# nv-tlabs/LION

Hardware: NVIDIA H100
Metric: shapes/sec (1000-step DDPM, 2048 latent pts, B=32) (higher is better)
Workload: dtype tf32 (fp32 storage/accumulate)

## Files before the change

include/lion_b200.h:

```cpp
#ifndef LION_B200_H
#define LION_B200_H
#include <stddef.h>
#ifdef __cplusplus
extern "C" {
#endif

typedef struct LionCtx LionCtx;
typedef struct LionModel LionModel;

int lion_version(void);
const char* lion_last_error(void);
int lion_ctx_create(int device, LionCtx** out);
int lion_ctx_destroy(LionCtx* ctx);
int lion_ctx_last_launches(LionCtx* ctx);
int lion_ctx_last_conv_group(LionCtx* ctx);
int lion_ctx_last_conv_stage_taps(LionCtx* ctx);
int lion_ctx_set_conv_whole_slabs(LionCtx* ctx, int on);
unsigned lion_ctx_generation(LionCtx* ctx);
int lion_ctx_timeline(LionCtx* ctx, unsigned long long* t_ns, char* names, int max_entries);
size_t lion_ctx_arena_bytes(LionCtx* ctx);
size_t lion_workspace_bytes(LionCtx* ctx);

int lion_avg_voxelize(const float* features, const int* coords, float* out, int* ind, int* cnt,
                      int B, int C, int N, int r, void* stream);
int lion_trilinear_devoxelize(const float* grid, const float* coords, float* out, int* inds, float* wgts,
                              int B, int C, int N, int r, int is_training, void* stream);
int lion_furthest_point_sampling(const float* coords, int* idx, int B, int N, int M, void* stream);
int lion_gather(const float* features, const int* idx, float* out, int B, int C, int N, int M, void* stream);
int lion_ball_query(const float* centers, const float* points, int* out, int B, int N, int M, float radius, int K,
                    void* stream);
int lion_grouping(const float* features, const int* idx, float* out, int B, int C, int N, int M, int U, void* stream);
int lion_three_nn_interpolate(const float* points, const float* centers, const float* centers_features, float* out,
                              int* idx, float* wgt, int B, int C, int N, int M, void* stream);
int lion_voxel_coords(const float* coords, float* norm_coords, int* vox, int B, int N, int r, int normalize, float eps,
                      void* stream);

int lion_avg_voxelize_backward(const float* grad_y , const int* ind , const int* cnt ,
                               float* grad_x , int B, int C, int N, int r, void* stream);
int lion_trilinear_devoxelize_backward(const float* grad_y , const int* inds , const float* wgts ,
                                       float* grad_x , int B, int C, int N, int r, void* stream);
int lion_grouping_backward(const float* grad_y , const int* idx , float* grad_x , int B, int C,
                           int N, int M, int U, void* stream);
int lion_three_nn_interpolate_backward(const float* grad_y , const int* idx , const float* wgt ,
                                       float* grad_x , int B, int C, int N, int M, void* stream);
int lion_gather_backward(const float* grad_y , const int* idx , float* grad_x , int B, int C, int N,
                         int M, void* stream);

enum { LION_KIND_UNET = 1, LION_KIND_PVCONV = 2, LION_KIND_SA = 3, LION_KIND_FP = 4, LION_KIND_ATTN = 5,
       LION_KIND_SHARED_MLP = 6, LION_KIND_GLOBAL_PRIOR = 7, LION_KIND_ADAGN = 8, LION_KIND_CONV3D = 9,
       LION_KIND_STYLE_ENC = 10 };
int lion_model_create(LionCtx* ctx, int kind, const int* desc, int ndesc, const float* const* params, int nparams,
                      LionModel** out);
int lion_model_destroy(LionModel* m);
int lion_model_refresh(LionModel* m);

int lion_unet_forward(LionModel* m, const float* x, const float* t, const float* style, const float* clip, float* out,
                      int B, int N, void* stream);
#define LION_FWD_CONV_FP16 1
int lion_unet_forward_flags(LionModel* m, const float* x, const float* t, const float* style, const float* clip, float* out,
                            int B, int N, int flags, void* stream);
int lion_unet_cache_style(LionModel* m, const float* style, const float* clip, int B, void* stream);
int lion_style_encoder_forward(LionModel* m, const float* x, float* out, int B, int N, void* stream);
int lion_pvconv_fwd(LionModel* m, const float* features, const float* coords, const float* style, float* out,
                    int B, int N, void* stream);
int lion_sa_module_fwd(LionModel* m, const float* features, const float* coords, const float* style,
                       float* out_features, float* out_coords, int B, int N, void* stream);
int lion_fp_module_fwd(LionModel* m, const float* points_coords, const float* centers_coords,
                       const float* centers_features, const float* points_features, const float* style, float* out,
                       int B, int N, int M, void* stream);
int lion_linear_attention_fwd(LionModel* m, const float* x, float* out, int B, int N, void* stream);
// ... 67 lines not shown
```

lion_b200/_lib.py:

```python
import ctypes as C
import os
import threading

import torch

_HERE = os.path.dirname(os.path.abspath(__file__))
LIB_PATH = os.path.join(_HERE, "csrc", "liblion_b200.so")


class LionError(RuntimeError):
    pass


_lib = None
_lock = threading.Lock()
c_f = C.c_void_p


def _proto(lib):
    i, f, sz, vp = C.c_int, C.c_float, C.c_size_t, C.c_void_p
    P = lambda *a: list(a)
    sig = {
        "lion_version": ([], i),
        "lion_last_error": ([], C.c_char_p),
        "lion_ctx_create": (P(i, C.POINTER(vp)), i),
        "lion_ctx_destroy": (P(vp), i),
        "lion_ctx_last_launches": (P(vp), i),
        "lion_ctx_last_conv_group": (P(vp), i),
        "lion_ctx_last_conv_stage_taps": (P(vp), i),
        "lion_ctx_set_conv_whole_slabs": (P(vp, i), i),
        "lion_ctx_arena_bytes": (P(vp), sz),
        "lion_ctx_generation": (P(vp), C.c_uint),
        "lion_ctx_timeline": (P(vp, vp, vp, i), i),
        "lion_avg_voxelize": (P(vp, vp, vp, vp, vp, i, i, i, i, vp), i),
        "lion_trilinear_devoxelize": (P(vp, vp, vp, vp, vp, i, i, i, i, i, vp), i),
        "lion_furthest_point_sampling": (P(vp, vp, i, i, i, vp), i),
        "lion_gather": (P(vp, vp, vp, i, i, i, i, vp), i),
        "lion_ball_query": (P(vp, vp, vp, i, i, i, f, i, vp), i),
        "lion_grouping": (P(vp, vp, vp, i, i, i, i, i, vp), i),
        "lion_three_nn_interpolate": (P(vp, vp, vp, vp, vp, vp, i, i, i, i, vp), i),
        "lion_voxel_coords": (P(vp, vp, vp, i, i, i, i, f, vp), i),
        "lion_avg_voxelize_backward": (P(vp, vp, vp, vp, i, i, i, i, vp), i),
        "lion_trilinear_devoxelize_backward": (P(vp, vp, vp, vp, i, i, i, i, vp), i),
        "lion_grouping_backward": (P(vp, vp, vp, i, i, i, i, i, vp), i),
        "lion_three_nn_interpolate_backward": (P(vp, vp, vp, vp, i, i, i, i, vp), i),
        "lion_gather_backward": (P(vp, vp, vp, i, i, i, i, vp), i),
        "lion_model_create": (P(vp, i, C.POINTER(i), i, C.POINTER(vp), i, C.POINTER(vp)), i),
        "lion_model_destroy": (P(vp), i),
        "lion_model_refresh": (P(vp), i),
        "lion_unet_forward": (P(vp, vp, vp, vp, vp, vp, i, i, vp), i),
        "lion_unet_forward_flags": (P(vp, vp, vp, vp, vp, vp, i, i, i, vp), i),
        "lion_unet_cache_style": (P(vp, vp, vp, i, vp), i),
        "lion_style_encoder_forward": (P(vp, vp, vp, i, i, vp), i),
        "lion_pvconv_fwd": (P(vp, vp, vp, vp, vp, i, i, vp), i),
        "lion_sa_module_fwd": (P(vp, vp, vp, vp, vp, vp, i, i, vp), i),
        "lion_fp_module_fwd": (P(vp, vp, vp, vp, vp, vp, vp, i, i, i, vp), i),
        "lion_linear_attention_fwd": (P(vp, vp, vp, i, i, vp), i),
        "lion_shared_mlp_fwd": (P(vp, vp, vp, vp, i, i, vp), i),
        "lion_global_prior_forward": (P(vp, vp, vp, vp, vp, i, vp), i),
        "lion_adagn_fwd": (P(vp, vp, vp, vp, i, i, vp), i),
        "lion_se3d_fwd": (P(vp, vp, vp, vp, vp, i, i, i, vp), i),
        "lion_swish_fwd": (P(vp, vp, sz, vp), i),
        "lion_ddpm_update": (P(vp, vp, vp, vp, vp, vp, f, sz, vp, i, vp), i),
        "lion_ddpm_set_step": (P(vp, vp, i, i, vp), i),
        "lion_ddpm_next_step": (P(vp, vp, i, vp), i),
        "lion_ddpm_fetch_noise": (P(vp, vp, vp, sz, vp), i),
        "lion_conv3d_gn_fwd": (P(vp, vp, vp, vp, vp, i, vp), i),
        "lion_conv3d_gn_fwd_flags": (P(vp, vp, vp, vp, vp, i, i, vp), i),
        "lion_pvconv_conv1_probe": (P(vp, vp, vp, i, vp, vp, vp, C.POINTER(i), i, i, vp), i),
        "lion_sa_mlp_probe": (P(vp, vp, vp, vp, i, vp, vp, vp, vp, vp, vp, C.POINTER(i), i, i, vp), i),
        "lion_pvconv_probe": (P(vp, vp, vp, vp, vp, vp, vp, vp, vp, vp, vp, vp, C.POINTER(i), i, i, vp), i),
        "lion_pvconv_probe_flags": (P(vp, vp, vp, vp, vp, vp, vp, vp, vp, vp, vp, vp, C.POINTER(i), i, i, i, vp), i),
        "lion_attention_probe": (P(vp, vp, vp, vp, vp, i, i, vp), i),
        "lion_global_prior_step": (P(vp, vp, vp, vp, vp, i, vp), i),
        "lion_workspace_bytes": (P(vp), sz),
        "lion_ddim_update": (P(vp, vp, vp, vp, vp, vp, sz, vp, vp), i),
        "lion_ddim_set_step": (P(vp, vp, vp, i, i, i, vp), i),
        "lion_ddim_next_step": (P(vp, vp, vp, i, i, vp), i),
        "lion_scheduler_step": (P(vp, vp, vp, vp, vp, vp, sz, vp), i),
        "lion_chamfer_forward": (P(vp, vp, vp, vp, vp, vp, i, i, i, vp), i),
        "lion_chamfer_pairwise": (P(vp, vp, vp, i, i, i, i, vp), i),
        "lion_chamfer_backward": (P(vp, vp, vp, vp, vp, vp, vp, vp, i, i, i, vp), i),
        "lion_emd_approx": (P(vp, vp, vp, i, i, i, vp), i),
# ... 174 lines not shown
```

lion_b200/csrc/common.cuh:

```cuda
#pragma once
#include <cuda_runtime.h>
#include <cstdint>
#include <cstdio>
#include <cstdarg>
#include <cstring>
#include <string>
#include <vector>
#include <mutex>

namespace lion {

enum : int { LION_OK = 0, LION_ERR_CUDA = -1, LION_ERR_ARG = -2, LION_ERR_OOM = -3, LION_ERR_STATE = -4 };

void set_error(const char* fmt, ...);
const char* get_error();

#define LION_CHECK_CUDA(expr)                                                          \
  do {                                                                                 \
    cudaError_t _e = (expr);                                                           \
    if (_e != cudaSuccess) {                                                           \
      lion::set_error("%s:%d: %s -> %s", __FILE__, __LINE__, #expr, cudaGetErrorString(_e)); \
      return lion::LION_ERR_CUDA;                                                      \
    }                                                                                  \
  } while (0)

#define LION_REQUIRE(cond, ...)                                                        \
  do {                                                                                 \
    if (!(cond)) {                                                                     \
      lion::set_error(__VA_ARGS__);                                                    \
      return lion::LION_ERR_ARG;                                                       \
    }                                                                                  \
  } while (0)

#define LION_TRY(expr)                                                                 \
  do {                                                                                 \
    int _r = (expr);                                                                   \
    if (_r != 0) return _r;                                                            \
  } while (0)

constexpr int LION_MAX_STAMPS = 256;
struct Ctx {
  int device = 0;
  int num_sms = 132;
  int l2_bytes = 50 << 20;
  cudaStream_t stream = nullptr;
  cudaStream_t aux = nullptr;
  char* base = nullptr;
  char* zgrid = nullptr;
  size_t zgrid_cap = 0, zgrid_need = 0;
  size_t cap = 0;
  size_t off = 0;
  size_t peak = 0;
  unsigned generation = 0;
  std::mutex* mu = nullptr;
  bool dry = false;
  int launches = 0;
  int conv_smem_cap = 0;
  int conv_group_blocks = 0;
  int conv_stage_taps = 0;
  bool conv_whole_slabs = false;
  unsigned long long* d_stamps = nullptr;
  int n_stamps = 0;
  char stamp_names[LION_MAX_STAMPS][24];

  void reset() { off = 0; peak = 0; launches = 0; zgrid_need = 0; n_stamps = 0; }
  void* alloc(size_t bytes) {
    size_t a = (off + 255) & ~size_t(255);
    off = a + bytes;
    if (off > peak) peak = off;
    if (dry) return (void*)(uintptr_t)(0x1000 + a);
    return base + a;
  }
  template <typename T> T* alloc_n(size_t n) { return (T*)alloc(n * sizeof(T)); }
  size_t mark() const { return off; }
  void release(size_t m) { off = m; }
};

int ctx_reserve(Ctx* c, size_t bytes);

#define LION_LAUNCH_ON(ctx, stream, kernel, grid, block, smem, ...)                    \
  do {                                                                                 \
    if (!(ctx)->dry) {                                                                 \
      kernel<<<(grid), (block), (smem), (stream)>>>(__VA_ARGS__);                      \
      (ctx)->launches++;                                                               \
    }                                                                                  \
  } while (0)
#define LION_LAUNCH(ctx, kernel, grid, block, smem, ...) LION_LAUNCH_ON(ctx, (ctx)->stream, kernel, grid, block, smem, __VA_ARGS__)

static __global__ void k_stamp(unsigned long long* p) {
  unsigned long long t;
  asm volatile("mov.u64 %0, %%globaltimer;" : "=l"(t));
  *p = t;
}
inline void stamp(Ctx* c, cudaStream_t s, const char* name, int idx = -1) {
  if (!c->d_stamps || c->dry || c->n_stamps >= LION_MAX_STAMPS) return;
  const char* pre = s == c->aux ? "aux:" : "";
  if (idx >= 0) snprintf(c->stamp_names[c->n_stamps], 24, "%s%s%d", pre, name, idx);
  else snprintf(c->stamp_names[c->n_stamps], 24, "%s%s", pre, name);
  k_stamp<<<1, 1, 0, s>>>(c->d_stamps + c->n_stamps);
  c->n_stamps++;
}

inline int memset_async(Ctx* c, void* p, int v, size_t bytes, cudaStream_t s) {
  if (c->dry || bytes == 0) return 0;
  LION_CHECK_CUDA(cudaMemsetAsync(p, v, bytes, s));
  return 0;
}
inline int memset_async(Ctx* c, void* p, int v, size_t bytes) { return memset_async(c, p, v, bytes, c->stream); }
inline int memcpy_d2d(Ctx* c, void* d, const void* s, size_t bytes) {
  if (c->dry || bytes == 0) return 0;
  LION_CHECK_CUDA(cudaMemcpyAsync(d, s, bytes, cudaMemcpyDeviceToDevice, c->stream));
  return 0;
}
// ... 62 lines not shown
```

lion_b200/csrc/conv_tc.cu:

```cuda
#include <algorithm>
#include <type_traits>
#include <cuda_fp16.h>

#include "common.cuh"
#include "model.cuh"
#include "wgmma.cuh"

namespace lion {
namespace tc {

using namespace sm90;

constexpr int CONSUMER_WARPS = 8;
constexpr int THREADS = 32 * CONSUMER_WARPS + 32;
__host__ __device__ constexpr int conv_threads(int BPW) { return BPW == 2 ? 32 * CONSUMER_WARPS + 128 : THREADS; }
constexpr int PRODUCER_REGS = 96, CONSUMER_REGS = 200;
constexpr int MAX_A_STAGES = 16;
constexpr int MAX_B_STAGES = 4;
constexpr int OCC_SMEM = 1024;
__host__ __device__ constexpr int tiles_per_item(int NT) { return NT <= 32 ? 4 : (NT <= 64 ? 2 : 1); }
constexpr int SMEM_BIAS = 128 * 4, SMEM_BARS = 64 * 8 + 128;
__host__ __device__ constexpr int smem_stat(int NT) { return CONSUMER_WARPS * 2 * NT * 4; }
__host__ __device__ constexpr int smem_pool(int NT, int TPG) { return TPG == 1 ? CONSUMER_WARPS * 2 * NT * 4 : 0; }
__host__ __device__ constexpr int smem_fixed(int NT, int TPG) {
  return SMEM_BIAS + smem_stat(NT) + smem_pool(NT, TPG) + SMEM_BARS + OCC_SMEM;
}

struct Params {
  const float4* in; const float* w; const float* bias; float4* out; double* ssum; double* ssq;
  int Gin, Gout_store, cout_pad;
  int rows;
  int p_begin, p_end;
  int ntile;
  int ntg, tpg;
  int tg_off[3];
  int tap_off[9];
  int r, rp, nzb, npl, nblk, ib;
  int halo;
  int KG, nchunk;
  int NT;
  int G;
  int B;
  int a_stage_bytes, b_stage_bytes, stage_rows;
  int a_stages;
  int b_stages;
  int tps;
  const unsigned char* occ;
  int occ_stride;
  float* pool_mm;
  int sched;
};

__host__ __device__ __forceinline__ int block_row(int k, int rp, int nzb, int npl) {
  const int x = k / npl, rem = k - x * npl, yb = rem / nzb, zb = rem - yb * nzb;
  return ((x + 1) * rp + 1 + 8 * yb) * rp + 1 + 8 * zb;
}

template <int KG, int TPG, int NT, int NB = 1, typename OP = float>
__device__ __forceinline__ void issue_stage(float (*d)[NT / 2], const uint32_t* a_addr, uint32_t b_addr, uint32_t a_pitch,
                                            uint32_t a_sbo, const int* tap_off) {
  const uint64_t b0 = make_desc(b_addr, NT * 16, 128);
  uint64_t a0[NB];
#pragma unroll
  for (int k = 0; k < NB; ++k) a0[k] = make_desc(a_addr[k], a_pitch, a_sbo);
#pragma unroll
  for (int t = 0; t < TPG; ++t) {
    const uint64_t toff = (uint64_t)(int64_t)(TPG == 1 ? 0 : tap_off[t]);
#pragma unroll
    for (int ks = 0; ks < KG / 2; ++ks)
#pragma unroll
      for (int k = 0; k < NB; ++k) {
        const uint64_t a = a0[k] + toff + (uint64_t)((ks * 2 * a_pitch) >> 4), b = b0 + (uint64_t)(((t * KG + ks * 2) * NT * 16) >> 4);
        if constexpr (std::is_same<OP, __half>::value) wgmma_f16<NT>(d[k], a, b, 1);
        else wgmma_tf32<NT>(d[k], a, b, 1);
      }
  }
}


struct Items {
  long long u, u_end; int ntile_total, B, G;
  int mode, m, q, n_p, n_q, c_i, i, big, k;
  __device__ __forceinline__ bool next(int& nt, long long& v0, int& ntile) {
    const long long per_nt = (long long)B * ntile_total;
    if (mode) {
      while (u >= u_end) {
        if (k >= m) return false;
        const int a0 = q * k / m, a1 = q * (k + 1) / m, b0 = (q + 1) * k / m, b1 = (q + 1) * (k + 1) / m;
        u = (long long)n_q * a0 + (long long)n_p * b0 + (long long)(i - c_i) * (a1 - a0) + (long long)c_i * (b1 - b0);
        u_end = u + (big ? b1 - b0 : a1 - a0);
        ++k;
      }
      nt = (int)(u / per_nt);
      v0 = u - (long long)nt * per_nt;
      const long long lim = (long long)(nt + 1) * per_nt;
      const long long e = u_end < lim ? u_end : lim;
      ntile = (int)(e - u);
      u = e;
      return true;
    }
    if (u >= u_end) return false;
    nt = (int)(u / per_nt);
    v0 = u - (long long)nt * per_nt;
    long long run = per_nt - v0;
    if (u_end - u < run) run = u_end - u;
    const long long k2 = (run + G - 1) / G;
    ntile = (int)((run + k2 - 1) / k2);
    u += ntile;
    return true;
  }
};
__device__ __forceinline__ Items make_items(long long U, int ntile_total, int B, int G, int sched) {
  const long long u_begin = U * blockIdx.x / gridDim.x, u_end = U * (blockIdx.x + 1) / gridDim.x;
  Items it{u_begin, u_end, ntile_total, B, G, 0, 0, 0, 0, 0, 0, 0, 0, 0};
  if (sched) {
    const int grid = (int)gridDim.x, q = (int)(U / grid), n_p = (int)(U - (long long)q * grid);
    const int tmax = q + (n_p ? 1 : 0);
    it.mode = 1; it.u = 0; it.u_end = 0;
    it.m = (tmax + G - 1) / G; it.q = q; it.n_p = n_p; it.n_q = grid - n_p;
    it.i = (int)blockIdx.x; it.c_i = (int)(u_begin - (long long)q * blockIdx.x);
    it.big = (int)(u_end - u_begin) > q; it.k = 0;
  }
  return it;
}

__device__ __forceinline__ void halo_mask(int p_lo, int rp, bool& ok_lo, bool& ok_hi) {
  const int p_hi = p_lo + 8;
  const int z0 = p_lo % rp, y0 = (p_lo / rp) % rp, z1 = p_hi % rp, y1 = (p_hi / rp) % rp;
  ok_lo = ok_lo && z0 >= 1 && z0 <= rp - 2 && y0 >= 1 && y0 <= rp - 2;
  ok_hi = ok_hi && z1 >= 1 && z1 <= rp - 2 && y1 >= 1 && y1 <= rp - 2;
}
template <int NT>
__device__ __forceinline__ void stat_add(float* s_stat, int cw, int lane, int col, float x0, float x1, float x2, float x3) {
  const float s0 = red8<0>(x0 + x2), s1 = red8<0>(x1 + x3);
  const float q0 = red8<0>(fmaf(x0, x0, x2 * x2)), q1 = red8<0>(fmaf(x1, x1, x3 * x3));
  if (lane < 4) {
    float* st = s_stat + (cw * 2) * NT + col;
    st[0] += s0; st[1] += s1; st[NT] += q0; st[NT + 1] += q1;
  }
}
template <int NT>
__device__ __forceinline__ void stat_flush(const Params& P, float* s_stat, int et, int b, int n0) {
  asm volatile("bar.sync 1, 256;" ::: "memory");
  if (et < NT) {
    float s = 0.f, qq = 0.f;
#pragma unroll
    for (int w = 0; w < CONSUMER_WARPS; ++w) {
      s += s_stat[(w * 2 + 0) * NT + et]; qq += s_stat[(w * 2 + 1) * NT + et];
      s_stat[(w * 2 + 0) * NT + et] = 0.0f; s_stat[(w * 2 + 1) * NT + et] = 0.0f;
    }
    atomicAdd(P.ssum + (size_t)b * P.cout_pad + n0 + et, (double)s);
    atomicAdd(P.ssq + (size_t)b * P.cout_pad + n0 + et, (double)qq);
  }
  asm volatile("bar.sync 1, 256;" ::: "memory");
}

template <int KG, int TPG, int NT, bool BLK, int BPW = 1, int TPS = TPG, typename OP = float>
__global__ void __launch_bounds__(conv_threads(BPW), 1) k_conv_tc(Params P) {
  constexpr int GT = BLK ? BPW : tiles_per_item(NT);
  constexpr int NTHR = conv_threads(BPW);
  constexpr bool SETREG = NTHR > THREADS;
  constexpr int NACC = NT / 2;
  constexpr int NPARTS = TPG / TPS;
  extern __shared__ __align__(128) uint8_t smem[];
  uint8_t* sA = smem;
  const int A_STAGES = P.a_stages;
  uint8_t* sB = sA + (size_t)A_STAGES * P.a_stage_bytes;
  const int B_STAGES = P.b_stages;
  float* s_bias = (float*)(sB + (size_t)B_STAGES * P.b_stage_bytes);
  float* s_stat = s_bias + 128;
  float* s_pool = s_stat + CONSUMER_WARPS * 2 * NT;
  uint64_t* bars = (uint64_t*)((uint8_t*)s_stat + smem_stat(NT) + smem_pool(NT, TPG));
  volatile uint32_t* s_skip = (volatile uint32_t*)(bars + 64);
  uint8_t* s_occ = (uint8_t*)(bars + 64) + 128;
  const int tid = threadIdx.x, warp = tid >> 5, lane = tid & 31;

  const uint32_t bar_full_a = smem_u32(bars), bar_empty_a = smem_u32(bars + MAX_A_STAGES);
  const uint32_t bar_full_b = smem_u32(bars + 2 * MAX_A_STAGES), bar_empty_b = smem_u32(bars + 2 * MAX_A_STAGES + MAX_B_STAGES);

  if (P.Gin % KG != 0)
    for (int i = tid; i < A_STAGES * P.a_stage_bytes / 16; i += NTHR) ((float4*)sA)[i] = make_float4(0.f, 0.f, 0.f, 0.f);
  for (int i = tid; i < CONSUMER_WARPS * 2 * NT; i += NTHR) s_stat[i] = 0.0f;
  if (tid == 0) {
    for (int i = 0; i < A_STAGES; ++i) { mbar_init(bar_full_a + 8 * i, 1); mbar_init(bar_empty_a + 8 * i, CONSUMER_WARPS); }
    for (int i = 0; i < B_STAGES; ++i) { mbar_init(bar_full_b + 8 * i, 1); mbar_init(bar_empty_b + 8 * i, CONSUMER_WARPS); }
    asm volatile("fence.mbarrier_init.release.cluster;" ::: "memory");
  }
  asm volatile("fence.proxy.async.shared::cta;" ::: "memory");
  __syncthreads();

  const int ntile_total = P.ntile;
  const int n_nt = P.cout_pad / P.NT;
  const long long U = (long long)n_nt * P.B * ntile_total;
  const Items items0 = make_items(U, ntile_total, P.B, P.G, P.sched);

  if (warp >= CONSUMER_WARPS) {
    if constexpr (SETREG) {
      regs_dec<PRODUCER_REGS>();
      if (warp > CONSUMER_WARPS) return;
    }
    uint32_t sa = 0, pa = 0, sb = 0, pb = 0;
    const uint32_t bytes = (uint32_t)P.stage_rows * 16u;
    const uint32_t sA_addr = smem_u32(sA), sB_addr = smem_u32(sB);
    Items items = items0;
    int nt, ntile;
    long long v0;
    int occ_shape = -1;
    const int slab_floats = P.tpg * KG * NT * 4;
    auto copy_weights = [&](const float* src) {
      mbar_wait<SETREG>(bar_empty_b + 8 * sb, pb ^ 1);
      if (lane == 0) {
        mbar_expect_tx(bar_full_b + 8 * sb, P.b_stage_bytes);
        bulk_g2s(sB_addr + sb * (uint32_t)P.b_stage_bytes, src, P.b_stage_bytes, bar_full_b + 8 * sb);
      }
      if (++sb == B_STAGES) { sb = 0; pb ^= 1; }
// ... 10 lines not shown
          const float* slab = wsrc + (size_t)(cc * P.ntg + tg) * slab_floats;
          copy_weights(slab);
          for (int j = 0; j < ntile; ++j) {
            const int bj = __shfl_sync(0xffffffffu, my_b, j), tj = __shfl_sync(0xffffffffu, my_t, j);
            long long row0;
            uint32_t cnt = (uint32_t)P.stage_rows;
            if (!BLK) {
              row0 = (long long)P.p_begin + (long long)tj * 128 - P.halo + P.tg_off[tg];
            } else {
              row0 = (long long)block_row(tj * P.ib, P.rp, P.nzb, P.npl) - P.rp - 1 + P.tg_off[tg];
              if (row0 + cnt > (long long)P.rows) cnt = (uint32_t)(P.rows - row0);
            }
            const float4* in_lane = P.in + ((size_t)bj * P.Gin + grp_lane) * P.rows;
            mbar_wait<SETREG>(bar_empty_a + 8 * sa, pa ^ 1);
            bool empty = false;
            if (may_skip) {
              const unsigned char* occ_b = P.occ + (size_t)bj * P.occ_stride;
              if (P.occ_stride <= OCC_SMEM) {
                if (occ_shape != bj) {
                  __syncwarp();
                  for (int k = lane; k < P.occ_stride; k += 32) s_occ[k] = __ldg(occ_b + k);
                  __syncwarp();
                  occ_shape = bj;
                }
                occ_b = s_occ;
              }
              long long lo = row0 < 0 ? 0 : row0, hi = row0 + cnt - 1;
              if (hi > P.rows - 1) hi = P.rows - 1;
              unsigned any = 0;
              for (int k = (int)(lo >> 6); k <= (int)(hi >> 6); ++k) any |= occ_b[k];
              empty = (any == 0);
            }
            const uint32_t full = bar_full_a + 8 * sa;
            if (lane == 0) {
              s_skip[sa] = empty ? 1u : 0u;
              if (empty) asm volatile("mbarrier.arrive.release.cta.shared::cta.b64 _, [%0];" ::"r"(full) : "memory");
              else mbar_expect_tx(full, cnt * 16u * kg_real);
            }
            __syncwarp();
            if (!empty && lane < kg_real)
              bulk_g2s(sA_addr + sa * (uint32_t)P.a_stage_bytes + lane * bytes, in_lane + row0, cnt * 16u, full);
            if (++sa == (uint32_t)A_STAGES) { sa = 0; pa ^= 1; }
          }
          for (int s = 1; s < NPARTS; ++s) copy_weights(slab + (size_t)s * (P.b_stage_bytes / 4));
        }
      }
    }
  } else {
    if constexpr (SETREG) regs_inc<CONSUMER_REGS>();
    const int cw = warp, wg = cw >> 2, wq = cw & 3;
    const int et = tid;
    const uint32_t a_pitch = (uint32_t)P.stage_rows * 16u;
    const uint32_t a_sbo = BLK ? (uint32_t)P.rp * 16u : 128u;
    const uint32_t a_ring = smem_u32(sA) + (BLK ? 0u : (uint32_t)(P.halo + 64 * wg) * 16u);
    const uint32_t b_ring = smem_u32(sB);
    const int r_lo = 64 * wg + 16 * wq + (lane >> 2);
    const int c_lo = 2 * (lane & 3);
    const bool odd = (lane & 1) != 0;
    float acc[GT][NACC];
    uint32_t sa = 0, pa = 0, sb = 0, pb = 0;
    Items items = items0;
    int nt, ntile;
    long long v0;
    auto release = [&](int& s, uint32_t bar0) {
      if (s >= 0) { if (lane == 0) mbar_arrive(bar0 + 8 * s); s = -1; }
    };
    while (items.next(nt, v0, ntile)) {
#pragma unroll
      for (int j = 0; j < GT; ++j)
#pragma unroll
        for (int i = 0; i < NACC; ++i) acc[j][i] = 0.0f;
      int g_f = 0, nbw = 0;
      uint32_t boff[GT];
      if (BLK) {
        const int g_b = (int)(v0 / ntile_total);
        g_f = (int)(v0 - (long long)g_b * ntile_total) * P.ib;
        const int nb = min(P.ib, P.nblk - g_f);
        nbw = (nb - wg + 1) / 2;
        const int s_f = block_row(g_f, P.rp, P.nzb, P.npl);
#pragma unroll
        for (int j = 0; j < GT; ++j) {
          const int k = 2 * j + wg < nb ? g_f + 2 * j + wg : g_f;
          boff[j] = (uint32_t)(block_row(k, P.rp, P.nzb, P.npl) - s_f + P.rp + 1) * 16u;
        }
      }
      int pend_a = -1, pend_b = -1;
      bool skip[BLK ? 1 : GT];
      for (int cc = 0; cc < P.nchunk; ++cc) {
        for (int tg = 0; tg < P.ntg; ++tg) {
          const uint32_t sa0 = sa, pa0 = pa;
#pragma unroll
          for (int s = 0; s < NPARTS; ++s) {
            mbar_wait<SETREG>(bar_full_b + 8 * sb, pb);
            const uint32_t b_addr = b_ring + sb * (uint32_t)P.b_stage_bytes;
            const int* toff = P.tap_off + s * TPS;
            bool issued = false;
            sa = sa0; pa = pa0;
#pragma unroll
            for (int j = 0; j < (BLK ? 1 : GT); ++j) {
              if (j < ntile) {
                if (s == 0) {
                  mbar_wait<SETREG>(bar_full_a + 8 * sa, pa);
                  skip[j] = s_skip[sa] != 0;
                  if (skip[j]) { int st = (int)sa; release(st, bar_empty_a); }
                }
                if (!skip[j]) {
                  const uint32_t a_addr = a_ring + sa * (uint32_t)P.a_stage_bytes;
                  wg_fence();
                  if (!BLK) {
                    issue_stage<KG, TPS, NT, 1, OP>(&acc[j], &a_addr, b_addr, a_pitch, a_sbo, toff);
                  } else {
                    uint32_t a_blk[GT];
#pragma unroll
                    for (int k = 0; k < GT; ++k) a_blk[k] = a_addr + boff[k];
                    issue_stage<KG, TPS, NT, GT, OP>(acc, a_blk, b_addr, a_pitch, a_sbo, toff);
                  }
                  wg_commit();
                  wg_wait<1>();
                  release(pend_a, bar_empty_a);
                  release(pend_b, bar_empty_b);
                  if (s == NPARTS - 1) pend_a = (int)sa;
                  issued = true;
                }
                if (++sa == (uint32_t)A_STAGES) { sa = 0; pa ^= 1; }
              }
            }
            if (pend_b >= 0) {
              wg_wait<0>();
              release(pend_a, bar_empty_a);
              release(pend_b, bar_empty_b);
            }
            if (issued) pend_b = (int)sb;
            else { int st = (int)sb; release(st, bar_empty_b); }
            if (++sb == B_STAGES) { sb = 0; pb ^= 1; }
          }
        }
      }
      wg_wait<0>();
      release(pend_a, bar_empty_a);
      release(pend_b, bar_empty_b);
#pragma unroll
      for (int j = 0; j < GT; ++j) fence_regs<NACC>(acc[j]);

      const int n0 = nt * NT;
      asm volatile("bar.sync 1, 256;" ::: "memory");
      if (et < NT) s_bias[et] = P.bias ? P.bias[n0 + et] : 0.0f;
      asm volatile("bar.sync 1, 256;" ::: "memory");
      int b = (int)(v0 / ntile_total);
#pragma unroll
      for (int j = 0; j < GT; ++j) {
        if (j < (BLK ? nbw : ntile)) {
          int tj = 0, p_lo, p_hi;
          bool ok_lo, ok_hi;
          bool in_lo, in_hi;
          if (!BLK) {
            const long long vj = v0 + j;
            const int bj = (int)(vj / ntile_total);
            tj = (int)(vj - (long long)bj * ntile_total);
            if (bj != b) { if (P.ssum) stat_flush<NT>(P, s_stat, et, b, n0); b = bj; }
            p_lo = P.p_begin + tj * 128 + r_lo; p_hi = p_lo + 8;
            in_lo = p_lo < P.p_end; in_hi = p_hi < P.p_end;
            ok_lo = in_lo; ok_hi = in_hi;
            if (TPG != 1) halo_mask(p_lo, P.rp, ok_lo, ok_hi);
          } else {
            const int k = g_f + 2 * j + wg, x = k / P.npl, rem = k - x * P.npl, yb = rem / P.nzb, zb = rem - yb * P.nzb;
            const int y = 1 + 8 * yb + 2 * wq, z = 1 + 8 * zb + (lane >> 2);
            p_lo = ((x + 1) * P.rp + y) * P.rp + z; p_hi = p_lo + P.rp;
            ok_lo = y <= P.r && z <= P.r; ok_hi = y + 1 <= P.r && z <= P.r;
            in_lo = ok_lo; in_hi = ok_hi;
          }
#pragma unroll
          for (int i = 0; i < NT / 8; ++i) {
            const int col = 8 * i + c_lo;
            const float x0 = ok_lo ? acc[j][4 * i + 0] + s_bias[col] : 0.0f, x1 = ok_lo ? acc[j][4 * i + 1] + s_bias[col + 1] : 0.0f;
            const float x2 = ok_hi ? acc[j][4 * i + 2] + s_bias[col] : 0.0f, x3 = ok_hi ? acc[j][4 * i + 3] + s_bias[col + 1] : 0.0f;
            if (P.ssum) stat_add<NT>(s_stat, cw, lane, col, x0, x1, x2, x3);
            if (TPG == 1 && P.pool_mm) {
              const float mn0 = red8<1>(fminf(x0, x2)), mn1 = red8<1>(fminf(x1, x3));
              const float mx0 = red8<2>(fmaxf(x0, x2)), mx1 = red8<2>(fmaxf(x1, x3));
              if (lane < 4) {
                float* sp = s_pool + (cw * 2) * NT + col;
                sp[0] = mn0; sp[1] = mn1; sp[NT] = mx0; sp[NT + 1] = mx1;
              }
            } else {
              const float y0 = __shfl_xor_sync(0xffffffffu, odd ? x0 : x2, 1);
              const float y1 = __shfl_xor_sync(0xffffffffu, odd ? x1 : x3, 1);
              const int g = (n0 + 8 * i + (lane & 2) * 2) >> 2;
              if (g < P.Gout_store) {
                float4* o = P.out + ((size_t)b * P.Gout_store + g) * P.rows;
                if (!odd && in_lo) o[p_lo] = make_float4(x0, x1, y0, y1);
                if (odd && in_hi) o[p_hi] = make_float4(y0, y1, x2, x3);
              }
            }
          }
          if (TPG == 1 && P.pool_mm) {
            const int bar_id = 2 + wg;
            asm volatile("bar.sync %0, 128;" ::"r"(bar_id) : "memory");
            const long long ncent = (long long)P.rows / 32;
            for (int e = et - 128 * wg; e < 2 * NT; e += 128) {
              const int k = e / NT, c = e - k * NT;
              const float* s0 = s_pool + ((4 * wg + 2 * k) * 2) * NT + c;
              const float* s1 = s0 + 2 * NT;
              const float mn = fminf(s0[0], s1[0]), mx = fmaxf(s0[NT], s1[NT]);
// ... 207 lines not shown
  P.ntile = ntile;
  P.a_stage_bytes = KG * P.stage_rows * 16;
  const double in_bytes = (double)B * Gin * geo.rows * 16.0;
  P.sched = w.ntaps == 27 && in_bytes > 1.6 * c->l2_bytes ? 1 : 0;
  auto ring = [&](int tps, int& b_stages) -> int {
    const long long stage = (long long)slab_bytes / tpg * tps;
    b_stages = tps == tpg ? 2 : tc::MAX_B_STAGES;
    if (blk && tps == tpg) {
      const long long limit = (c->conv_smem_cap > 0 ? c->conv_smem_cap : 227LL * 1024) - (long long)fixed;
      while (b_stages < tc::MAX_B_STAGES && (limit - (b_stages + 1) * stage) / P.a_stage_bytes >= std::max(4, b_stages + 1))
        ++b_stages;
    }
    int a_stages = (int)((227LL * 1024 - (long long)fixed - b_stages * stage) / P.a_stage_bytes);
    if (c->conv_smem_cap > 0 && a_stages >= 5) {
      const int capped = (int)(((long long)c->conv_smem_cap - (long long)fixed - b_stages * stage) / P.a_stage_bytes);
      if (capped >= 4 && capped < a_stages) a_stages = capped;
    }
    a_stages = std::min(a_stages, tc::MAX_A_STAGES);
    return a_stages >= 2 ? a_stages : 0;
  };
  int b_whole = 0, b_parts = 0;
  const int a_whole = ring(tpg, b_whole);
  const int a_parts = blk && !c->conv_whole_slabs ? ring(3, b_parts) : 0;
  const bool parts = a_parts > a_whole && a_parts >= P.G + 1;
  if (!parts && !a_whole) {
    set_error("conv_tc: shared memory cannot hold the operand pipeline (N=%d, KG=%d)", NT, KG); return LION_ERR_ARG;
  }
  P.tps = parts ? 3 : tpg;
  P.b_stage_bytes = slab_bytes / tpg * P.tps;
  P.b_stages = parts ? b_parts : b_whole;
  const int a_stages = parts ? a_parts : a_whole;
  P.a_stages = a_stages;
  const int b_stages = P.b_stages;
  if (!blk && P.occ && a_stages < 2 * P.G) P.occ = nullptr;
  size_t smem = (size_t)a_stages * P.a_stage_bytes + (size_t)b_stages * P.b_stage_bytes + fixed;
  if (smem > 227 * 1024) { set_error("conv_tc: %zu bytes of shared memory needed", smem); return LION_ERR_ARG; }
  auto grid_for = [&](int nt_per_shape) {
    long long n_units = (long long)nt_per_shape * n_tiles_n * B;
    long long per_cta = (n_units + c->num_sms - 1) / c->num_sms;
    return (int)((n_units + per_cta - 1) / per_cta);
  };
  const int grid = grid_for(ntile);
  tc::Params S = P;
  if (blk && ssum) {
    P.ssum = nullptr; P.ssq = nullptr;
    S.ntile = ntile_rows; S.G = tc::tiles_per_item(NT);
  }
  auto stats = [&]() -> int {
    if (!(blk && ssum)) return 0;
    LION_LAUNCH(c, tc::k_conv_stats<128>, grid_for(ntile_rows), 256, 0, S);
    return check_launch(c, "conv_tc stats");
  };
  const int bpw = blk ? P.ib / 2 : 1;
  c->conv_group_blocks = blk ? P.ib : 0;
  c->conv_stage_taps = P.tps;
#define CONV_TC_CASE_OP(kg, tpg_, nt_, blk_, bpw_, tps_, op)                                              \
  if (f16 == std::is_same<op, __half>::value && KG == kg && tpg == tpg_ && NT == nt_ && blk == blk_ && bpw == bpw_ && P.tps == tps_) { \
    static DevOnce attr_once;                                                                             \
    if (attr_once.need()) {                                                                               \
      LION_CHECK_CUDA(cudaFuncSetAttribute(tc::k_conv_tc<kg, tpg_, nt_, blk_, bpw_, tps_, op>, cudaFuncAttributeMaxDynamicSharedMemorySize, 227 * 1024)); \
    }                                                                                                     \
    LION_LAUNCH(c, (tc::k_conv_tc<kg, tpg_, nt_, blk_, bpw_, tps_, op>), grid, tc::conv_threads(bpw_), smem, P); \
    LION_TRY(check_launch(c, "conv_tc"));                                                                 \
    return stats();                                                                                       \
  }
#define CONV_TC_CASE(kg, tpg_, nt_, blk_, bpw_, tps_) CONV_TC_CASE_OP(kg, tpg_, nt_, blk_, bpw_, tps_, float)
#define CONV_TC_NT(kg, tpg_) CONV_TC_CASE(kg, tpg_, 32, false, 1, tpg_) CONV_TC_CASE(kg, tpg_, 64, false, 1, tpg_) CONV_TC_CASE(kg, tpg_, 96, false, 1, tpg_)
#define CONV_TC_BLK(kg, bpw_) CONV_TC_CASE(kg, 9, 128, true, bpw_, 9) CONV_TC_CASE(kg, 9, 128, true, bpw_, 3)
  CONV_TC_NT(2, 1) CONV_TC_NT(4, 1) CONV_TC_NT(8, 1) CONV_TC_NT(2, 9) CONV_TC_NT(4, 9) CONV_TC_NT(8, 9)
  CONV_TC_CASE(2, 1, 128, false, 1, 1) CONV_TC_CASE(4, 1, 128, false, 1, 1) CONV_TC_CASE(8, 1, 128, false, 1, 1)
  CONV_TC_BLK(2, 1) CONV_TC_BLK(4, 1) CONV_TC_BLK(2, 2) CONV_TC_BLK(4, 2)
  CONV_TC_CASE_OP(4, 9, 32, false, 1, 9, __half) CONV_TC_CASE_OP(8, 9, 64, false, 1, 9, __half)
  CONV_TC_CASE_OP(4, 9, 128, true, 1, 9, __half) CONV_TC_CASE_OP(4, 9, 128, true, 1, 3, __half)
  CONV_TC_CASE_OP(4, 9, 128, true, 2, 9, __half) CONV_TC_CASE_OP(4, 9, 128, true, 2, 3, __half)
#undef CONV_TC_NT
#undef CONV_TC_BLK
#undef CONV_TC_CASE
#undef CONV_TC_CASE_OP
  set_error("conv_tc: no %s kernel for N=%d, KG=%d, %d taps, %d per weight stage", f16 ? "FP16" : "TF32", NT, KG, tpg, P.tps);
  return LION_ERR_ARG;
}

}
```

lion_b200/csrc/net.cu:

```cuda
#include <algorithm>
#include <deque>
#include <memory>
#include <cstdlib>
#include <cmath>
#include "common.cuh"
#include "packed_kernels.cuh"
#include "model.cuh"
#include "../../include/lion_b200.h"

namespace lion {

static thread_local char g_err[1024] = "";
void set_error(const char* fmt, ...) {
  va_list ap;
  va_start(ap, fmt);
  vsnprintf(g_err, sizeof(g_err), fmt, ap);
  va_end(ap);
}
const char* get_error() { return g_err; }

int ctx_reserve(Ctx* c, size_t bytes) {
  if (bytes <= c->cap) return 0;
  cudaStreamCaptureStatus st = cudaStreamCaptureStatusNone;
  cudaStreamIsCapturing(c->stream, &st);
// ... 1030 lines not shown
    }
  }
  return 0;
}

}

using namespace lion;

struct LionCtx { Ctx c; std::mutex mu; };
struct LionModel { Model m; };

extern "C" int lion_version(void) { return 100; }
extern "C" const char* lion_last_error(void) { return get_error(); }

extern "C" int lion_ctx_create(int device, LionCtx** out) {
  LION_REQUIRE(out, "lion_ctx_create: null out");
  LION_CHECK_CUDA(cudaSetDevice(device));
  LionCtx* h = new LionCtx();
  h->c.device = device;
  h->c.mu = &h->mu;
  cudaDeviceProp prop;
  LION_CHECK_CUDA(cudaGetDeviceProperties(&prop, device));
  h->c.num_sms = prop.multiProcessorCount;
  h->c.l2_bytes = prop.l2CacheSize;
  LION_CHECK_CUDA(cudaStreamCreateWithFlags(&h->c.aux, cudaStreamNonBlocking));
  { const char* e = getenv("LION_TIMELINE");
    if (e && atoi(e) != 0) LION_CHECK_CUDA(cudaMalloc(&h->c.d_stamps, LION_MAX_STAMPS * sizeof(unsigned long long))); }
  if (prop.major != 9 || prop.minor != 0) {
    set_error("lion_b200 is built for sm_90a only; device %d is sm_%d%d", device, prop.major, prop.minor);
    delete h;
    return LION_ERR_STATE;
  }
  *out = h;
  return 0;
}
extern "C" int lion_ctx_destroy(LionCtx* h) {
  if (!h) return 0;
  if (h->c.base) cudaFree(h->c.base);
  if (h->c.zgrid) cudaFree(h->c.zgrid);
  if (h->c.aux) cudaStreamDestroy(h->c.aux);
  if (h->c.d_stamps) cudaFree(h->c.d_stamps);
  delete h;
  return 0;
}
extern "C" int lion_ctx_last_launches(LionCtx* h) { return h ? h->c.launches : 0; }
extern "C" int lion_ctx_last_conv_group(LionCtx* h) { return h ? h->c.conv_group_blocks : 0; }
extern "C" int lion_ctx_last_conv_stage_taps(LionCtx* h) { return h ? h->c.conv_stage_taps : 0; }
extern "C" int lion_ctx_set_conv_whole_slabs(LionCtx* h, int on) {
  LION_REQUIRE(h, "lion_ctx_set_conv_whole_slabs: null context");
  h->c.conv_whole_slabs = on != 0;
  return 0;
}
extern "C" unsigned lion_ctx_generation(LionCtx* h) { return h ? h->c.generation : 0; }
extern "C" int lion_ctx_timeline(LionCtx* h, unsigned long long* t_ns, char* names, int max_entries) {
  LION_REQUIRE(h && t_ns && names && max_entries >= 0, "lion_ctx_timeline: null argument");
  if (!h->c.d_stamps) { set_error("lion_ctx_timeline: the context was created without LION_TIMELINE=1"); return LION_ERR_STATE; }
  int n = h->c.n_stamps < max_entries ? h->c.n_stamps : max_entries;
  LION_CHECK_CUDA(cudaSetDevice(h->c.device));
  LION_CHECK_CUDA(cudaDeviceSynchronize());
  LION_CHECK_CUDA(cudaMemcpy(t_ns, h->c.d_stamps, (size_t)n * sizeof(unsigned long long), cudaMemcpyDeviceToHost));
  for (int i = 0; i < n; ++i) memcpy(names + (size_t)i * 24, h->c.stamp_names[i], 24);
  return n;
}
extern "C" size_t lion_ctx_arena_bytes(LionCtx* h) { return h ? h->c.cap : 0; }
extern "C" size_t lion_workspace_bytes(LionCtx* h) { return h ? h->c.cap + h->c.zgrid_cap : 0; }

extern "C" int lion_model_create(LionCtx* ctx, int kind, const int* desc, int ndesc, const float* const* params,
                                 int nparams, LionModel** out) {
  LION_REQUIRE(ctx && out && (desc || ndesc == 0) && (params || nparams == 0), "lion_model_create: null argument");
  LION_CHECK_CUDA(cudaSetDevice(ctx->c.device));
  std::unique_ptr<LionModel> h(new LionModel());
  Model* m = &h->m;
  m->ctx = &ctx->c; m->kind = kind;
  m->desc.assign(desc, desc + ndesc);
  m->params.assign(params, params + nparams);
  for (int i = 0; i < nparams; ++i) LION_REQUIRE(params[i], "lion_model_create: parameter %d is null", i);
  Cursor cur{m->params.data(), nparams};
  const std::vector<int>& d = m->desc;
  auto need = [&](int n) { return (int)d.size() >= n; };
  switch (kind) {
    case LION_KIND_UNET: LION_TRY(build_unet(m, cur)); break;
    case LION_KIND_PVCONV: {
      LION_REQUIRE(need(5), "pvconv descriptor: [cin, cout, r, attn, style_dim]");
      m->S = d[4] > 0 ? d[4] : 4;
      m->block.reset(new Block()); m->block->kind = kind;
      LION_TRY(make_pvconv(m, m->block->pv, cur, d[0], d[1], d[2], d[3] != 0, d[4] == 0));
      break;
    }
    case LION_KIND_SA: {
      LION_REQUIRE(need(6) && need(6 + d[5]), "sa descriptor: [cfeat, m, radius_bits, k, style_dim, n, outs...]");
      m->S = d[4] > 0 ? d[4] : 4;
      m->block.reset(new Block()); m->block->kind = kind;
      LION_TRY(make_sa(m, m->block->sa, cur, d[0], d[1], bits_to_float(d[2]), d[3], std::vector<int>(d.begin() + 6, d.begin() + 6 + d[5]), d[4] == 0));
      break;
    }
    case LION_KIND_FP: {
      LION_REQUIRE(need(4) && need(4 + d[3]), "fp descriptor: [cc, cp, style_dim, n, outs...]");
      m->S = d[2];
      m->block.reset(new Block()); m->block->kind = kind;
      LION_TRY(make_fp(m, m->block->fp, cur, d[0], d[1], std::vector<int>(d.begin() + 4, d.begin() + 4 + d[3])));
      break;
    }
    case LION_KIND_ATTN: {
      LION_REQUIRE(need(2), "attention descriptor: [C, heads]");
      LION_REQUIRE(d[0] % 4 == 0, "attention: C must be a multiple of 4");
// ... 494 lines not shown
```

Measured before the change: 3.053.

## Map voxel rows onto wgmma N dimension for 64-channel TF32 3x3x3 convs

For TF32 3x3x3 sparse-voxel convs with 64 output channels, the wgmma operands are swapped: the 64 output channels sit on M and 128 voxel rows on N. Each warpgroup then issues one N=128 instruction per tile instead of one N=64 instruction. This is meant to make better use of the tensor cores for narrow-channel layers. It needs a new epilogue that masks halo rows with shuffles, reduces statistics and writes transposed output. It also waits on wgmma fully (wait 0) after each stage, which removes overlap, and each warpgroup skips the tiles it does not own.

```diff
diff --git a/include/lion_b200.h b/include/lion_b200.h
--- a/include/lion_b200.h
+++ b/include/lion_b200.h
@@ -16,6 +16,8 @@
 int lion_ctx_last_conv_group(LionCtx* ctx);
 int lion_ctx_last_conv_stage_taps(LionCtx* ctx);
 int lion_ctx_set_conv_whole_slabs(LionCtx* ctx, int on);
+int lion_ctx_set_conv_rows_on_m(LionCtx* ctx, int on);
+int lion_ctx_last_conv_rows_on_n(LionCtx* ctx);
 unsigned lion_ctx_generation(LionCtx* ctx);
 int lion_ctx_timeline(LionCtx* ctx, unsigned long long* t_ns, char* names, int max_entries);
 size_t lion_ctx_arena_bytes(LionCtx* ctx);
diff --git a/lion_b200/_lib.py b/lion_b200/_lib.py
--- a/lion_b200/_lib.py
+++ b/lion_b200/_lib.py
@@ -29,6 +29,8 @@
         "lion_ctx_last_conv_group": (P(vp), i),
         "lion_ctx_last_conv_stage_taps": (P(vp), i),
         "lion_ctx_set_conv_whole_slabs": (P(vp, i), i),
+        "lion_ctx_set_conv_rows_on_m": (P(vp, i), i),
+        "lion_ctx_last_conv_rows_on_n": (P(vp), i),
         "lion_ctx_arena_bytes": (P(vp), sz),
         "lion_ctx_generation": (P(vp), C.c_uint),
         "lion_ctx_timeline": (P(vp, vp, vp, i), i),
diff --git a/lion_b200/csrc/common.cuh b/lion_b200/csrc/common.cuh
--- a/lion_b200/csrc/common.cuh
+++ b/lion_b200/csrc/common.cuh
@@ -59,6 +59,8 @@
   int conv_group_blocks = 0;
   int conv_stage_taps = 0;
   bool conv_whole_slabs = false;
+  bool conv_rows_on_m = false;
+  bool conv_rows_on_n = false;
   unsigned long long* d_stamps = nullptr;
   int n_stamps = 0;
   char stamp_names[LION_MAX_STAMPS][24];
diff --git a/lion_b200/csrc/conv_tc.cu b/lion_b200/csrc/conv_tc.cu
--- a/lion_b200/csrc/conv_tc.cu
+++ b/lion_b200/csrc/conv_tc.cu
@@ -56,9 +56,10 @@
   return ((x + 1) * rp + 1 + 8 * yb) * rp + 1 + 8 * zb;
 }
 
-template <int KG, int TPG, int NT, int NB = 1, typename OP = float>
-__device__ __forceinline__ void issue_stage(float (*d)[NT / 2], const uint32_t* a_addr, uint32_t b_addr, uint32_t a_pitch,
-                                            uint32_t a_sbo, const int* tap_off) {
+template <int KG, int TPG, int NT, int NB = 1, typename OP = float, bool RN = false>
+__device__ __forceinline__ void issue_stage(float (*d)[RN ? 64 : NT / 2], const uint32_t* a_addr, uint32_t b_addr,
+                                            uint32_t a_pitch, uint32_t a_sbo, const int* tap_off) {
+  static_assert(!RN || (NT == 64 && NB == 1 && std::is_same<OP, float>::value), "rows on N: 64 channels, TF32, one tile");
   const uint64_t b0 = make_desc(b_addr, NT * 16, 128);
   uint64_t a0[NB];
 #pragma unroll
@@ -71,7 +72,8 @@
 #pragma unroll
       for (int k = 0; k < NB; ++k) {
         const uint64_t a = a0[k] + toff + (uint64_t)((ks * 2 * a_pitch) >> 4), b = b0 + (uint64_t)(((t * KG + ks * 2) * NT * 16) >> 4);
-        if constexpr (std::is_same<OP, __half>::value) wgmma_f16<NT>(d[k], a, b, 1);
+        if constexpr (RN) wgmma_tf32<128>(d[k], b, a, 1);
+        else if constexpr (std::is_same<OP, __half>::value) wgmma_f16<NT>(d[k], a, b, 1);
         else wgmma_tf32<NT>(d[k], a, b, 1);
       }
   }
@@ -155,12 +157,103 @@
   asm volatile("bar.sync 1, 256;" ::: "memory");
 }
 
-template <int KG, int TPG, int NT, bool BLK, int BPW = 1, int TPS = TPG, typename OP = float>
+template <int NT>
+__device__ __forceinline__ int epilogue_rn(const Params& P, float* d, const float* s_bias, float* s_stat, long long v0,
+                                           int ntile, int ntile_total, int n0, int wg, int wq, int lane, int et) {
+  const int q = lane & 3, s = (lane >> 2) & 3;
+  const int c0 = 16 * wq + (lane >> 2);
+  int b = (int)(v0 / ntile_total);
+  const bool mine = wg < ntile;
+  const long long vj = v0 + (mine ? wg : 0);
+  const int bj = (int)(vj / ntile_total), tj = (int)(vj - (long long)bj * ntile_total);
+  const int p0 = P.p_begin + tj * 128 + 2 * q;
+  if (mine) {
+    int z = p0 % P.rp, y = (p0 / P.rp) % P.rp;
+    const float bias0 = s_bias[c0], bias1 = s_bias[c0 + 8];
+#pragma unroll
+    for (int i = 0; i < 16; ++i) {
+#pragma unroll
+      for (int e = 0; e < 2; ++e) {
+        int ze = z + e, ye = y;
+        if (ze == P.rp) { ze = 0; ye = ye + 1 == P.rp ? 0 : ye + 1; }
+        const bool ok = p0 + 8 * i + e < P.p_end && ze >= 1 && ze <= P.rp - 2 && ye >= 1 && ye <= P.rp - 2;
+        d[4 * i + e] = ok ? d[4 * i + e] + bias0 : 0.0f;
+        d[4 * i + 2 + e] = ok ? d[4 * i + 2 + e] + bias1 : 0.0f;
+      }
+      z += 8;
+      while (z >= P.rp) { z -= P.rp; if (++y == P.rp) y = 0; }
+    }
+  }
+  if (P.ssum) {
+    float sm[8][2], sq[8][2];
+#pragma unroll
+    for (int g = 0; g < 8; ++g)
+#pragma unroll
+      for (int h = 0; h < 2; ++h) {
+        const float* lo = d + 8 * g + 2 * h;
+        const float* hi = lo + 4;
+        float t = (lo[0] + hi[0]) + (lo[1] + hi[1]);
+        float u = fmaf(lo[0], lo[0], hi[0] * hi[0]) + fmaf(lo[1], lo[1], hi[1] * hi[1]);
+        t += __shfl_xor_sync(0xffffffffu, t, 1); u += __shfl_xor_sync(0xffffffffu, u, 1);
+        t += __shfl_xor_sync(0xffffffffu, t, 2); u += __shfl_xor_sync(0xffffffffu, u, 2);
+        sm[g][h] = t; sq[g][h] = u;
+      }
+    auto add = [&]() {
+#pragma unroll
+      for (int g = 0; g < 8; ++g)
+        if (q == g >> 1)
+#pragma unroll
+          for (int h = 0; h < 2; ++h) {
+            s_stat[(g * 2) * NT + c0 + 8 * h] += sm[g][h];
+            s_stat[(g * 2 + 1) * NT + c0 + 8 * h] += sq[g][h];
+          }
+    };
+    if (mine && wg == 0) add();
+    asm volatile("bar.sync 1, 256;" ::: "memory");
+    if (ntile > 1) {
+      const int b1 = (int)((v0 + 1) / ntile_total);
+      if (b1 != b) { stat_flush<NT>(P, s_stat, et, b, n0); b = b1; }
+      if (mine && wg == 1) add();
+    }
+  } else if (ntile > 1) {
+    b = (int)((v0 + 1) / ntile_total);
+  }
+  if (mine) {
+#pragma unroll
+    for (int h = 0; h < 2; ++h) {
+      const int g4 = (n0 + 16 * wq + 8 * h + 4 * (lane >> 4)) >> 2;
+      float4* o = P.out + ((size_t)bj * P.Gout_store + g4) * P.rows;
+#pragma unroll
+      for (int a = 0; a < 8; ++a) {
+        const float* v = d + 8 * a + 2 * h;
+        float A0[2], A1[2];
+#pragma unroll
+        for (int pp = 0; pp < 2; ++pp) {
+          const float keep = (s & 1) ? v[4 * pp + 1] : v[4 * pp], send = (s & 1) ? v[4 * pp] : v[4 * pp + 1];
+          const float recv = __shfl_xor_sync(0xffffffffu, send, 4);
+          A0[pp] = (s & 1) ? recv : keep;
+          A1[pp] = (s & 1) ? keep : recv;
+        }
+        const int hs = s >> 1;
+        const float k0 = hs ? A0[1] : A0[0], k1 = hs ? A1[1] : A1[0];
+        const float r0 = __shfl_xor_sync(0xffffffffu, hs ? A0[0] : A0[1], 8);
+        const float r1 = __shfl_xor_sync(0xffffffffu, hs ? A1[0] : A1[1], 8);
+        const int p = p0 + 16 * a + 8 * hs + (s & 1);
+        if (p < P.p_end && g4 < P.Gout_store) o[p] = hs ? make_float4(r0, r1, k0, k1) : make_float4(k0, k1, r0, r1);
+      }
+    }
+  }
+  return b;
+}
+
+template <int KG, int TPG, int NT, bool BLK, int BPW = 1, int TPS = TPG, typename OP = float, bool RN = false>
 __global__ void __launch_bounds__(conv_threads(BPW), 1) k_conv_tc(Params P) {
-  constexpr int GT = BLK ? BPW : tiles_per_item(NT);
+  static_assert(!RN || (!BLK && TPG == 9 && NT == 64), "rows on N: 3x3x3 row tiles with 64 output channels");
+  constexpr int NTI = BLK ? 1 : tiles_per_item(NT);
+  constexpr int GT = BLK ? BPW : (RN ? 1 : NTI);
   constexpr int NTHR = conv_threads(BPW);
   constexpr bool SETREG = NTHR > THREADS;
-  constexpr int NACC = NT / 2;
+  constexpr int NACC = RN ? 64 : NT / 2;
   constexpr int NPARTS = TPG / TPS;
   extern __shared__ __align__(128) uint8_t smem[];
   uint8_t* sA = smem;
@@ -277,7 +370,7 @@
     const int et = tid;
     const uint32_t a_pitch = (uint32_t)P.stage_rows * 16u;
     const uint32_t a_sbo = BLK ? (uint32_t)P.rp * 16u : 128u;
-    const uint32_t a_ring = smem_u32(sA) + (BLK ? 0u : (uint32_t)(P.halo + 64 * wg) * 16u);
+    const uint32_t a_ring = smem_u32(sA) + (BLK ? 0u : (uint32_t)(P.halo + (RN ? 0 : 64 * wg)) * 16u);
     const uint32_t b_ring = smem_u32(sB);
     const int r_lo = 64 * wg + 16 * wq + (lane >> 2);
     const int c_lo = 2 * (lane & 3);
@@ -310,7 +403,7 @@
         }
       }
       int pend_a = -1, pend_b = -1;
-      bool skip[BLK ? 1 : GT];
+      bool skip[NTI];
       for (int cc = 0; cc < P.nchunk; ++cc) {
         for (int tg = 0; tg < P.ntg; ++tg) {
           const uint32_t sa0 = sa, pa0 = pa;
@@ -322,17 +415,19 @@
             bool issued = false;
             sa = sa0; pa = pa0;
 #pragma unroll
-            for (int j = 0; j < (BLK ? 1 : GT); ++j) {
+            for (int j = 0; j < NTI; ++j) {
               if (j < ntile) {
                 if (s == 0) {
                   mbar_wait<SETREG>(bar_full_a + 8 * sa, pa);
-                  skip[j] = s_skip[sa] != 0;
+                  skip[j] = s_skip[sa] != 0 || (RN && j != wg);
                   if (skip[j]) { int st = (int)sa; release(st, bar_empty_a); }
                 }
                 if (!skip[j]) {
                   const uint32_t a_addr = a_ring + sa * (uint32_t)P.a_stage_bytes;
                   wg_fence();
-                  if (!BLK) {
+                  if constexpr (RN) {
+                    issue_stage<KG, TPS, NT, 1, OP, RN>(acc, &a_addr, b_addr, a_pitch, a_sbo, toff);
+                  } else if constexpr (!BLK) {
                     issue_stage<KG, TPS, NT, 1, OP>(&acc[j], &a_addr, b_addr, a_pitch, a_sbo, toff);
                   } else {
                     uint32_t a_blk[GT];
@@ -341,7 +436,7 @@
                     issue_stage<KG, TPS, NT, GT, OP>(acc, a_blk, b_addr, a_pitch, a_sbo, toff);
                   }
                   wg_commit();
-                  wg_wait<1>();
+                  wg_wait<RN ? 0 : 1>();
                   release(pend_a, bar_empty_a);
                   release(pend_b, bar_empty_b);
                   if (s == NPARTS - 1) pend_a = (int)sa;
@@ -357,6 +452,10 @@
             }
             if (issued) pend_b = (int)sb;
             else { int st = (int)sb; release(st, bar_empty_b); }
+            if constexpr (RN) {
+              release(pend_a, bar_empty_a);
+              release(pend_b, bar_empty_b);
+            }
             if (++sb == B_STAGES) { sb = 0; pb ^= 1; }
           }
         }
@@ -372,8 +471,9 @@
       if (et < NT) s_bias[et] = P.bias ? P.bias[n0 + et] : 0.0f;
       asm volatile("bar.sync 1, 256;" ::: "memory");
       int b = (int)(v0 / ntile_total);
-#pragma unroll
-      for (int j = 0; j < GT; ++j) {
+      if constexpr (RN) b = epilogue_rn<NT>(P, acc[0], s_bias, s_stat, v0, ntile, ntile_total, n0, wg, wq, lane, et);
+#pragma unroll
+      for (int j = 0; j < (RN ? 0 : GT); ++j) {
         if (j < (BLK ? nbw : ntile)) {
           int tj = 0, p_lo, p_hi;
           bool ok_lo, ok_hi;
@@ -687,27 +787,31 @@
     return check_launch(c, "conv_tc stats");
   };
   const int bpw = blk ? P.ib / 2 : 1;
+  const bool rn = w.ntaps == 27 && NT == 64 && !f16 && !c->conv_rows_on_m;
+  c->conv_rows_on_n = rn;
   c->conv_group_blocks = blk ? P.ib : 0;
   c->conv_stage_taps = P.tps;
-#define CONV_TC_CASE_OP(kg, tpg_, nt_, blk_, bpw_, tps_, op)                                              \
-  if (f16 == std::is_same<op, __half>::value && KG == kg && tpg == tpg_ && NT == nt_ && blk == blk_ && bpw == bpw_ && P.tps == tps_) { \
+#define CONV_TC_CASE_OP(kg, tpg_, nt_, blk_, bpw_, tps_, op, rn_)                                         \
+  if (f16 == std::is_same<op, __half>::value && KG == kg && tpg == tpg_ && NT == nt_ && blk == blk_ && bpw == bpw_ && P.tps == tps_ && rn == rn_) { \
     static DevOnce attr_once;                                                                             \
     if (attr_once.need()) {                                                                               \
-      LION_CHECK_CUDA(cudaFuncSetAttribute(tc::k_conv_tc<kg, tpg_, nt_, blk_, bpw_, tps_, op>, cudaFuncAttributeMaxDynamicSharedMemorySize, 227 * 1024)); \
+      LION_CHECK_CUDA(cudaFuncSetAttribute(tc::k_conv_tc<kg, tpg_, nt_, blk_, bpw_, tps_, op, rn_>, cudaFuncAttributeMaxDynamicSharedMemorySize, 227 * 1024)); \
     }                                                                                                     \
-    LION_LAUNCH(c, (tc::k_conv_tc<kg, tpg_, nt_, blk_, bpw_, tps_, op>), grid, tc::conv_threads(bpw_), smem, P); \
+    LION_LAUNCH(c, (tc::k_conv_tc<kg, tpg_, nt_, blk_, bpw_, tps_, op, rn_>), grid, tc::conv_threads(bpw_), smem, P); \
     LION_TRY(check_launch(c, "conv_tc"));                                                                 \
     return stats();                                                                                       \
   }
-#define CONV_TC_CASE(kg, tpg_, nt_, blk_, bpw_, tps_) CONV_TC_CASE_OP(kg, tpg_, nt_, blk_, bpw_, tps_, float)
+#define CONV_TC_CASE(kg, tpg_, nt_, blk_, bpw_, tps_) CONV_TC_CASE_OP(kg, tpg_, nt_, blk_, bpw_, tps_, float, false)
 #define CONV_TC_NT(kg, tpg_) CONV_TC_CASE(kg, tpg_, 32, false, 1, tpg_) CONV_TC_CASE(kg, tpg_, 64, false, 1, tpg_) CONV_TC_CASE(kg, tpg_, 96, false, 1, tpg_)
 #define CONV_TC_BLK(kg, bpw_) CONV_TC_CASE(kg, 9, 128, true, bpw_, 9) CONV_TC_CASE(kg, 9, 128, true, bpw_, 3)
   CONV_TC_NT(2, 1) CONV_TC_NT(4, 1) CONV_TC_NT(8, 1) CONV_TC_NT(2, 9) CONV_TC_NT(4, 9) CONV_TC_NT(8, 9)
   CONV_TC_CASE(2, 1, 128, false, 1, 1) CONV_TC_CASE(4, 1, 128, false, 1, 1) CONV_TC_CASE(8, 1, 128, false, 1, 1)
   CONV_TC_BLK(2, 1) CONV_TC_BLK(4, 1) CONV_TC_BLK(2, 2) CONV_TC_BLK(4, 2)
-  CONV_TC_CASE_OP(4, 9, 32, false, 1, 9, __half) CONV_TC_CASE_OP(8, 9, 64, false, 1, 9, __half)
-  CONV_TC_CASE_OP(4, 9, 128, true, 1, 9, __half) CONV_TC_CASE_OP(4, 9, 128, true, 1, 3, __half)
-  CONV_TC_CASE_OP(4, 9, 128, true, 2, 9, __half) CONV_TC_CASE_OP(4, 9, 128, true, 2, 3, __half)
+  CONV_TC_CASE_OP(4, 9, 32, false, 1, 9, __half, false) CONV_TC_CASE_OP(8, 9, 64, false, 1, 9, __half, false)
+  CONV_TC_CASE_OP(4, 9, 128, true, 1, 9, __half, false) CONV_TC_CASE_OP(4, 9, 128, true, 1, 3, __half, false)
+  CONV_TC_CASE_OP(4, 9, 128, true, 2, 9, __half, false) CONV_TC_CASE_OP(4, 9, 128, true, 2, 3, __half, false)
+  CONV_TC_CASE_OP(2, 9, 64, false, 1, 9, float, true) CONV_TC_CASE_OP(4, 9, 64, false, 1, 9, float, true)
+  CONV_TC_CASE_OP(8, 9, 64, false, 1, 9, float, true)
 #undef CONV_TC_NT
 #undef CONV_TC_BLK
 #undef CONV_TC_CASE
diff --git a/lion_b200/csrc/net.cu b/lion_b200/csrc/net.cu
--- a/lion_b200/csrc/net.cu
+++ b/lion_b200/csrc/net.cu
@@ -1106,6 +1106,12 @@
   h->c.conv_whole_slabs = on != 0;
   return 0;
 }
+extern "C" int lion_ctx_set_conv_rows_on_m(LionCtx* h, int on) {
+  LION_REQUIRE(h, "lion_ctx_set_conv_rows_on_m: null context");
+  h->c.conv_rows_on_m = on != 0;
+  return 0;
+}
+extern "C" int lion_ctx_last_conv_rows_on_n(LionCtx* h) { return h ? (int)h->c.conv_rows_on_n : 0; }
 extern "C" unsigned lion_ctx_generation(LionCtx* h) { return h ? h->c.generation : 0; }
 extern "C" int lion_ctx_timeline(LionCtx* h, unsigned long long* t_ns, char* names, int max_entries) {
   LION_REQUIRE(h && t_ns && names && max_entries >= 0, "lion_ctx_timeline: null argument");
```

New measurement: 3.116 (median of 6 runs). +2.1%, better.
